# Shuijing725/CrowdNav_Prediction_AttnGraph

Hardware: NVIDIA H100
Metric: env_steps_per_s_ppo_rollout (higher is better)
Workload: dtype f32

## Files before the change

### crowdnav_prediction_attngraph_b200/_capi.py

```python
import ctypes as C
import os

_PKG = os.path.dirname(os.path.abspath(__file__))
LIB_PATH = os.path.join(_PKG, "libcrowdnav_b200.so")


class CnConfig(C.Structure):
    _fields_ = [(n, C.c_int32) for n in (
        "num_envs", "nenv_total", "rank_offset", "seed", "human_num", "predict_steps", "const_vel",
        "randomize_attributes", "random_goal_changing", "end_goal_changing", "sort_humans", "device",
        "phase", "val_size", "test_size", "human_num_range", "human_policy")] + \
        [("robot_policy", C.c_int16), ("robot_visible", C.c_int16)] + \
        [(n, C.c_double) for n in (
            "time_step", "time_limit", "pred_timestep", "circle_radius", "arena_size",
            "discomfort_dist", "discomfort_penalty_factor", "success_reward", "collision_penalty",
            "human_radius", "human_v_pref", "human_fov", "robot_radius", "robot_v_pref", "robot_fov",
            "sensor_range", "goal_change_chance", "orca_neighbor_dist", "orca_safety_space",
            "orca_time_horizon", "sf_A", "sf_B", "sf_KI")]


class CnObsPtrs(C.Structure):
    _fields_ = [("robot_node", C.c_void_p), ("temporal_edges", C.c_void_p), ("spatial_edges", C.c_void_p),
                ("detected_human_num", C.c_void_p), ("visible_masks", C.c_void_p)]

# ... 13 lines not shown


class CnActPtrs(C.Structure):
    _fields_ = [(n, C.c_void_p) for n in (
        "robot_node", "temporal_edges", "spatial_edges", "detected_human_num", "h_in", "masks", "noise",
        "value", "action", "log_prob", "h_out", "action_mean")]


class CnDsrnnConfig(C.Structure):
    _fields_ = [("num_envs", C.c_int32), ("human_num", C.c_int32), ("input_size", C.c_int32), ("device", C.c_int32)]


class CnDsrnnActPtrs(C.Structure):
    _fields_ = [(n, C.c_void_p) for n in (
        "robot_node", "temporal_edges", "spatial_edges", "h_in", "edge_h_in", "masks", "noise",
        "value", "action", "log_prob", "h_out", "edge_h_out", "action_mean")]


ABI_VERSION = 3

EXPORTS = [
    "cn_last_error", "cn_abi_version", "cn_env_create", "cn_env_destroy", "cn_env_reset", "cn_env_step",
    "cn_env_step_host", "cn_env_state_bytes", "cn_env_state_copy", "cn_env_launch_count", "cn_env_profile", "cn_env_stage_ms",
    "cn_policy_create", "cn_policy_destroy", "cn_policy_set_param", "cn_policy_finalize",
    "cn_policy_act", "cn_policy_launch_count", "cn_policy_last_rows", "cn_policy_profile", "cn_policy_stage_count",
    "cn_policy_stage_name", "cn_policy_handle_stage_name", "cn_policy_stage_ms", "cn_copy_segments", "cn_fetch_sync",
    "cn_gst_create", "cn_gst_destroy", "cn_gst_set_param", "cn_gst_finalize", "cn_gst_reset", "cn_gst_step",
    "cn_gst_launch_count",
    "cn_update_linear_saved_bytes", "cn_update_linear_ws_bytes", "cn_update_linear_fwd", "cn_update_linear_bwd",
    "cn_update_attn_fwd", "cn_update_attn_bwd", "cn_update_gru_fwd", "cn_update_gru_bwd",
    "cn_dsrnn_create", "cn_dsrnn_destroy", "cn_dsrnn_set_param", "cn_dsrnn_finalize", "cn_dsrnn_act",
    "cn_dsrnn_launch_count", "cn_dsrnn_profile", "cn_dsrnn_stage_count", "cn_dsrnn_stage_name", "cn_dsrnn_stage_ms",
    "cn_env_create_collect", "cn_env_reset_collect", "cn_env_step_collect", "cn_recorder_create", "cn_recorder_destroy",
    "cn_recorder_append", "cn_recorder_pending", "cn_recorder_flush", "cn_write_rows_txt", "cn_format_rows",
]

_lib = None


def config_from_dict(d):
    cfg = CnConfig()
    for name, _ in CnConfig._fields_:
        setattr(cfg, name, d[name])
    return cfg


# ... 40 lines not shown
    lib.cn_gst_create.restype = C.c_int
    lib.cn_gst_create.argtypes = [C.c_int, C.c_int, C.c_int, C.c_double, C.c_double, C.c_double, C.c_int, C.POINTER(C.c_void_p)]
    lib.cn_gst_destroy.argtypes = [C.c_void_p]
    lib.cn_gst_set_param.restype = C.c_int
    lib.cn_gst_set_param.argtypes = [C.c_void_p, C.c_char_p, C.c_void_p, C.c_size_t]
    lib.cn_gst_finalize.restype = C.c_int
    lib.cn_gst_finalize.argtypes = [C.c_void_p]
    lib.cn_gst_reset.restype = C.c_int
    lib.cn_gst_reset.argtypes = [C.c_void_p, C.c_void_p]
    lib.cn_gst_step.restype = C.c_int
    lib.cn_gst_step.argtypes = [C.c_void_p] * 7 + [C.c_void_p]
    lib.cn_gst_launch_count.restype = C.c_int64
    lib.cn_gst_launch_count.argtypes = [C.c_void_p]
    lib.cn_copy_segments.restype = C.c_int
    lib.cn_copy_segments.argtypes = [C.POINTER(CnCopySeg), C.c_int, C.c_int, C.c_void_p]
    lib.cn_fetch_sync.restype = C.c_int
    lib.cn_fetch_sync.argtypes = [C.c_void_p, C.c_void_p, C.c_size_t, C.c_int, C.c_void_p]
    lib.cn_env_launch_count.restype = C.c_int64
    lib.cn_env_launch_count.argtypes = [C.c_void_p]
    lib.cn_env_profile.restype = C.c_int
    lib.cn_env_profile.argtypes = [C.c_void_p, C.c_int]
    lib.cn_env_stage_ms.restype = C.c_int
    lib.cn_env_stage_ms.argtypes = [C.c_void_p, C.POINTER(C.c_float)]
    lib.cn_policy_create.argtypes = [C.POINTER(CnPolicyConfig), C.POINTER(C.c_void_p)]
    lib.cn_policy_destroy.argtypes = [C.c_void_p]
    lib.cn_policy_set_param.argtypes = [C.c_void_p, C.c_char_p, C.c_void_p, C.c_size_t]
    lib.cn_policy_finalize.argtypes = [C.c_void_p, C.c_void_p]
    lib.cn_policy_act.argtypes = [C.c_void_p, C.POINTER(CnActPtrs), C.c_void_p]
    lib.cn_policy_launch_count.restype = C.c_int64
    lib.cn_policy_launch_count.argtypes = [C.c_void_p]
    lib.cn_policy_last_rows.restype = C.c_int64
    lib.cn_policy_last_rows.argtypes = [C.c_void_p]
    lib.cn_policy_profile.argtypes = [C.c_void_p, C.c_int]
    lib.cn_policy_stage_count.restype = C.c_int
    lib.cn_policy_stage_name.restype = C.c_char_p
    lib.cn_policy_stage_name.argtypes = [C.c_int]
    lib.cn_policy_handle_stage_name.restype = C.c_char_p
    lib.cn_policy_handle_stage_name.argtypes = [C.c_void_p, C.c_int]
    lib.cn_policy_stage_ms.argtypes = [C.c_void_p, C.c_void_p, C.c_int]
    lib.cn_dsrnn_create.argtypes = [C.POINTER(CnDsrnnConfig), C.POINTER(C.c_void_p)]
    lib.cn_dsrnn_destroy.argtypes = [C.c_void_p]
    lib.cn_dsrnn_set_param.argtypes = [C.c_void_p, C.c_char_p, C.c_void_p, C.c_size_t]
    lib.cn_dsrnn_finalize.argtypes = [C.c_void_p, C.c_void_p]
    lib.cn_dsrnn_act.argtypes = [C.c_void_p, C.POINTER(CnDsrnnActPtrs), C.c_void_p]
    lib.cn_dsrnn_launch_count.restype = C.c_int64
    lib.cn_dsrnn_launch_count.argtypes = [C.c_void_p]
# ... 40 lines not shown
```

### crowdnav_prediction_attngraph_b200/csrc/cn_env_kernels.cu

```cuda
#include <cuda_runtime.h>
#include <stdio.h>
#include <stdlib.h>
#include <string.h>
#include <string>
#include <vector>
#include <map>

#include "../../include/crowdnav_b200.h"
#include "cn_env_core.cuh"
#include "cn_host_util.h"

namespace {

struct EnvSmemLayout {
  size_t per_env;
  size_t off_dbl;
  size_t off_flt;
  size_t off_u8;
};

__host__ __device__ inline size_t align16(size_t x) { return (x + 15) & ~(size_t)15; }

__host__ __device__ inline EnvSmemLayout env_layout(int H, bool lean, bool sf = false) {
  EnvSmemLayout L;
// ... 54 lines not shown

__device__ __forceinline__ void cn_sf_obs_lookahead(const CnParams& p, CnEnvSh* s, int h, bool live, float* row) {
  const bool seen = live && s->visr[h] != 0;
  double spx = 0.0, spy = 0.0, swx = 0.0, swy = 0.0, pen = 0.0;
  if (live) { spx = s->px[h]; spy = s->py[h]; swx = s->wx[h]; swy = s->wy[h]; }
  for (int t = 1; t <= p.lookahead_steps; ++t) {
    __syncthreads();
    CnD2 v = {0.0, 0.0};
    if (live) v = cn_sf_velocity(p, *s, h, false);
    __syncthreads();
    if (live) {
      const double x = s->px[h] + v.x * p.time_step, y = s->py[h] + v.y * p.time_step;
      s->px[h] = x; s->py[h] = y; s->wx[h] = v.x; s->wy[h] = v.y;
      if (seen && t % p.pred_interval == 0) cn_truth_row(p, *s, x, y, t / p.pred_interval, row, pen);
    }
  }
  __syncthreads();
  if (live) {
    s->px[h] = spx; s->py[h] = spy; s->wx[h] = swx; s->wy[h] = swy;
    if (seen) s->t1[h] = pen;
  }
}

template <int MAXH, int MAXW, bool ROBOT, bool VIS, bool COLLECT = false, bool SFLA = false, bool TRUTH = false>
__global__ void __launch_bounds__(288, 2) cn_env_step_kernel(CnParams p, CnState g, const float* __restrict__ action,
                                                          CnObs ob, CnStepOut out, int epb, int line_cap, int mode) {
  extern __shared__ __align__(16) unsigned char smem[];
  const int H = p.H;
  const int le = threadIdx.x / H;
  const int h = threadIdx.x - le * H;
  const int e = (le < epb) ? g.perm[blockIdx.x * epb + le] : p.N;
  const bool active = (le < epb) && (e < p.N);
  const EnvSmemLayout L = env_layout(H, true, p.social_force != 0);
  CnEnvSh* s = nullptr;
  if (le < epb) {
    s = reinterpret_cast<CnEnvSh*>(smem + (size_t)le * L.per_env);
    if (h == 0 && e < p.N) env_view(smem + (size_t)le * L.per_env, L, H, true, g, e, p.social_force != 0);
  }
  __syncthreads();
  const int warp = threadIdx.x >> 5, lane = threadIdx.x & 31;
  float4* lines_smem = reinterpret_cast<float4*>(smem + align16((size_t)epb * L.per_env));
  const int lstride = epb * H;
  CnWarpLines W;
  W.smem0 = lines_smem + warp * 32;
  W.stride = lstride;
  W.cap = line_cap;
  W.ovf_stride = g.ovf_stride;
  W.ovf0 = reinterpret_cast<float4*>(g.line_ovf) + ((size_t)blockIdx.x * blockDim.x + warp * 32) * g.ovf_stride;
  const int half = lane >> 4;
  const CnCoop hco = {lane & 15, 16, nullptr, nullptr, half ? 0xffff0000u : 0x0000ffffu, half << 4};
  CnLineStore proj;
  proj.base = lines_smem + (size_t)line_cap * lstride + (size_t)(2 * warp + half) * H;
  proj.stride = 1; proj.cap = H; proj.ovf = nullptr;
  unsigned char* lp3_q = reinterpret_cast<unsigned char*>(lines_smem + (size_t)line_cap * lstride +
                                                          (size_t)(blockDim.x >> 4) * H);
  if (threadIdx.x == 0) { reinterpret_cast<int*>(lp3_q)[0] = 0; reinterpret_cast<int*>(lp3_q)[1] = 0; }
  const CnCoop co = {lane, 32, nullptr, nullptr};

  if (mode == 1) {
    if (active && h == 0) { s->done = 1; s->info = 0; s->reward = 0.0; s->reset_flag = 0; s->nvis = 0; s->goal_flag = 0; s->lp3_cost = 0; s->hn = 0; }
  } else if (active) {
    cn_phase_load<MAXH, ROBOT>(p, g, *s, e, h, mode == 3 ? nullptr : action);
  }
  __syncthreads();
  const bool live = active && h < s->hn;
  int* lp3_count = reinterpret_cast<int*>(lp3_q);
  int* lp3_head = lp3_count + 1;
  unsigned short* lp3_tasks = reinterpret_cast<unsigned short*>(lp3_count + 2);
  auto orca_solve = [&](bool lv, bool use_fov, CnF2& result, int& nl, int& fail) {
    nl = 0; fail = -1;
    float vmax = 0.0f;
    CnF2 pref = f2(0.0f, 0.0f);
    result = f2(0.0f, 0.0f);
    if (lv) cn_orca_build<MAXH, VIS>(p, g, *s, e, h, W.of(lane), nl, vmax, pref, use_fov, mode == 3 ? (uint8_t)2 : (uint8_t)1);
    __syncwarp();
    cn_orca_lp2_warp(hco, W, nl, vmax, pref, result, fail);
    if (fail >= 0) {
      s->nvx[h] = result.x; s->nvy[h] = result.y;
      reinterpret_cast<int*>(&s->t0[h])[0] = nl | (fail << 8);
      reinterpret_cast<float*>(&s->t0[h])[1] = vmax;
      lp3_tasks[atomicAdd(lp3_count, 1)] = (unsigned short)threadIdx.x;
    }
    __syncthreads();
    const int ntask = *lp3_count;
    for (;;) {
      int t = 0;
      if (hco.lane == 0) t = atomicAdd(lp3_head, 1);
      t = __shfl_sync(hco.mask, t, hco.base);
      if (t >= ntask) break;
      const int owner = lp3_tasks[t];
      const int ole = owner / H, oh = owner - ole * H;
      CnEnvSh* os = reinterpret_cast<CnEnvSh*>(smem + (size_t)ole * L.per_env);
      const int packed = reinterpret_cast<const int*>(&os->t0[oh])[0];
      const float ovmax = reinterpret_cast<const float*>(&os->t0[oh])[1];
      CnF2 ores = f2(os->nvx[oh], os->nvy[oh]);
      CnLineStore ol;
      ol.base = lines_smem + owner; ol.stride = lstride; ol.cap = line_cap;
      ol.ovf = reinterpret_cast<float4*>(g.line_ovf) + ((size_t)blockIdx.x * blockDim.x + owner) * g.ovf_stride;
      cn_lp3_coop(hco, ol, packed & 0xff, packed >> 8, ovmax, ores, proj);
      if (hco.lane == 0) { os->nvx[oh] = ores.x; os->nvy[oh] = ores.y; }
    }
    __syncthreads();
    if (fail >= 0) result = f2(s->nvx[h], s->nvy[h]);
    if (threadIdx.x == 0) { *lp3_count = 0; *lp3_head = 0; }
  };
  if (mode != 1 && p.social_force) {
    if (live) cn_sf_action<VIS>(p, g, *s, e, h);
    if (SFLA && (!TRUTH || p.test_phase)) cn_sf_lookahead(p, g, s, e, h, live);
  } else if (mode == 2) {
    if (live) {
      const size_t i = cn_idx(p, e, h);
      const int nlf = g.pre_nlf[i];
      cn_orca_finish(p, g, *s, e, h, f2(g.pre_vx[i], g.pre_vy[i]), nlf & 0xff, (nlf >> 8) - 1);
      if (g.sim_exists[i] >= 2) g.sim_exists[i] = 1;
    }
  } else if (mode != 1) {
    CnF2 result; int nl, fail;
    orca_solve(live, true, result, nl, fail);
    if (live && fail >= 0) atomicAdd(&s->lp3_cost, 1);
    if (mode == 3) {
      if (live) {
        const size_t i = cn_idx(p, e, h);
        g.pre_vx[i] = result.x; g.pre_vy[i] = result.y; g.pre_nlf[i] = nl | ((fail + 1) << 8);
      }
      __syncthreads();
      if (active && h == 0) g.lp_cost[e] = s->lp3_cost;
      return;
    }
    if (p.test_phase && !COLLECT) {
      double spx = 0, spy = 0, lx = 0, ly = 0;
      float svx = 0, svy = 0, lvx = 0, lvy = 0;
      bool vis_prev = false;
      if (live) {
        spx = s->px[h]; spy = s->py[h]; svx = s->vx[h]; svy = s->vy[h];
        lx = spx; ly = spy; lvx = svx; lvy = svy;
        vis_prev = g.vis[cn_idx(p, e, h)] != 0;
      }
      CnLookahead la; la.min_rd = INFINITY; la.pen = 0.0;
      CnF2 lres = f2(0.0f, 0.0f); int lnl = 0, lfail = -1;
      for (int t = 1; t <= p.lookahead_steps; ++t) {
        __syncthreads();
        if (live) {
          s->px[h] = lx; s->py[h] = ly; s->fx[h] = (float)lx; s->fy[h] = (float)ly; s->vx[h] = lvx; s->vy[h] = lvy;
        }
        __syncthreads();
        orca_solve(live, false, lres, lnl, lfail);
        lx = lx + (double)lres.x * p.time_step; ly = ly + (double)lres.y * p.time_step;
        lvx = lres.x; lvy = lres.y;
        if (live && t % p.pred_interval == 0) cn_lookahead_accumulate(p, *s, vis_prev, lx, ly, t / p.pred_interval, la);
      }
      __syncthreads();
      if (live) {
        s->px[h] = spx; s->py[h] = spy; s->fx[h] = (float)spx; s->fy[h] = (float)spy; s->vx[h] = svx; s->vy[h] = svy;
      }
      __syncthreads();
      if (live) {
        cn_orca_finish(p, g, *s, e, h, result, nl, fail);
        cn_orca_diag(p, g, e, h, lres, lnl, lfail);
        s->t0[h] = la.min_rd; s->t1[h] = la.pen;
      }
    } else if (live) {
      cn_orca_finish(p, g, *s, e, h, result, nl, fail);
    }
  }
  __syncthreads();
  if (mode != 1 && active && h == 0) {
    if (COLLECT) cn_collect_reward(p, g, *s, e, out);
    else cn_phase_reward(p, g, *s, e, out);
  }
  if (COLLECT && mode == 1 && active && h == 0) g.rgoal_due[e] = 0;
  __syncthreads();
  if (active) {
    if (s->done) cn_install_env(p, g, *s, e, h);
    else if (live) cn_phase_integrate(p, *s, h);
  }
  __syncthreads();
  if (p.hrange > 0) {
    if (mode != 1 && active && h == 0 && cn_add_remove_due(p, g, *s, e)) cn_phase_add_remove(p, g, *s, e);
    __syncthreads();
  }
  float row[MAXW];
  if (COLLECT) {
    __shared__ uint32_t leaving[(288 + 31) / 32];
    const bool seen_before = active && h < s->hn && g.vis[cn_idx(p, e, h)] != 0;
    if (active) cn_phase_obs_a<MAXW>(p, g, *s, e, h, row);
    __syncthreads();
    const uint32_t b = __ballot_sync(0xffffffffu, seen_before && !s->reset_flag && !s->visr[h]);
    if (lane == 0) leaving[warp] = b;
    __syncthreads();
    if (active) cn_collect_ids(p, g, *s, e, h, leaving, le * H, ob);
    __syncthreads();
    if (active) cn_phase_store(p, g, *s, e, h);
    if (active && h == 0) {
      cn_collect_ids_done(p, g, *s, e, leaving, le * H);
      int evt = cn_event_flag(p, g, *s, e);
      if (evt == 0 && g.rgoal_due[e]) evt = 1;
      g.evt[e] = (uint8_t)evt;
      if (mode != 2) g.lp_cost[e] = s->lp3_cost;
    }
// ... 25 lines not shown
        lvx = lres.x; lvy = lres.y;
        if (seen && t % p.pred_interval == 0) cn_truth_row(p, *s, lx, ly, t / p.pred_interval, row, pen);
      }
      __syncthreads();
      if (olive) {
        s->px[h] = spx; s->py[h] = spy; s->fx[h] = (float)spx; s->fy[h] = (float)spy; s->vx[h] = svx; s->vy[h] = svy;
        s->t0[h] = key;
        if (seen) s->t1[h] = pen;
        if (p.lookahead_steps > 0) cn_orca_diag(p, g, e, h, lres, lnl, lfail);
      }
    }
    __syncthreads();
  }
  if (active) cn_phase_obs_b(p, g, *s, e, h, row, ob);
  __syncthreads();
  if (active) {
    cn_phase_obs_c(p, *s, e, h, ob);
    cn_phase_store(p, g, *s, e, h);
  }
  if (active && h == 0) {
    g.evt[e] = (uint8_t)cn_event_flag(p, g, *s, e);
    if (mode != 2) g.lp_cost[e] = s->lp3_cost;
  }
}

#define CN_EVENT_WARPS 4
template <bool COLLECT = false>
__global__ void __launch_bounds__(CN_EVENT_WARPS * 32) cn_env_event_kernel(CnParams p, CnState g, int force,
                                                                           size_t per_warp_bytes) {
  extern __shared__ __align__(16) unsigned char smem[];
  const int warp = threadIdx.x >> 5, lane = threadIdx.x & 31;
  const int e = blockIdx.x * CN_EVENT_WARPS + warp;
  if (e >= p.N) return;
  const int evt = force ? 2 : g.evt[e];
  if (evt == 0) return;
  const int H = p.H;
  const EnvSmemLayout L = env_layout(H, false, p.social_force != 0);
  unsigned char* base = smem + (size_t)warp * per_warp_bytes;
  CnEnvSh* s = reinterpret_cast<CnEnvSh*>(base);
  if (lane == 0) env_view(base, L, H, false, g, e, p.social_force != 0);
  __syncwarp();
  uint32_t* key = reinterpret_cast<uint32_t*>(base + L.per_env);
  const CnCoop co = {lane, 32, nullptr, reinterpret_cast<float*>(key + 624)};
  bool deferred;
  if (evt == 2) {
    deferred = cn_prepare_env(p, g, *s, e, key, co, p.defer_tries);
// ... 95 lines not shown
  } else {
    const unsigned char* s1 = reinterpret_cast<const unsigned char*>(sg.src);
    unsigned char* d1 = reinterpret_cast<unsigned char*>(sg.dst);
    for (size_t i = tid; i < sg.bytes; i += nth) d1[i] = s1[i];
  }
}

struct Field {
  void* ptr;
  size_t bytes;
};

}

struct cn_env {
  cn_config cfg;
  CnParams p;
  CnState g;
  int device;
  int epb;
  int threads;
  size_t smem_bytes;
  int line_cap;
  size_t reset_warp_bytes;
  int heavy_grid;
  size_t heavy_smem;
  int maxh;
  int64_t launches;
  std::map<std::string, Field> fields;
  std::vector<void*> allocs;
  cudaStream_t side;
  cudaEvent_t ev_step, ev_side;
  bool profile = false;
  cudaEvent_t pev[5] = {nullptr, nullptr, nullptr, nullptr, nullptr};
  bool side_pending;
  bool use_side;
  bool presolve;
  bool presolved;
  bool balance;
  bool prep_dirty;
  float* d_action;
  cn_obs_ptrs d_obs;
  cn_step_ptrs d_out;
};

namespace {
// ... 33 lines not shown
}

KernelFn pick_kernel_sfla(int maxh) {
  if (maxh <= 32) return cn_env_step_kernel<32, 16, true, true, false, true>;
  if (maxh <= 64) return cn_env_step_kernel<64, 16, true, true, false, true>;
  return cn_env_step_kernel<128, 16, true, true, false, true>;
}

template <bool SF>
KernelFn pick_kernel_truth(int maxh) {
  if (maxh <= 32) return cn_env_step_kernel<32, 16, false, true, false, SF, true>;
  if (maxh <= 64) return cn_env_step_kernel<64, 16, false, true, false, SF, true>;
  return cn_env_step_kernel<128, 16, false, true, false, SF, true>;
}

KernelFn pick_kernel(const CnParams& p, int maxh) {
  if (p.collect) return pick_kernel_collect(maxh);
  if (p.const_vel == 2) return p.social_force ? pick_kernel_truth<true>(maxh) : pick_kernel_truth<false>(maxh);
  if (p.social_force && p.test_phase) return pick_kernel_sfla(maxh);
  const bool robot = p.robot_policy != 0, vis = p.robot_visible != 0;
  return vis ? pick_kernel_vis<true>(maxh, robot) : pick_kernel_vis<false>(maxh, robot);
}

CnObs to_obs(const cn_obs_ptrs* o) {
  CnObs ob;
  ob.robot_node = o->robot_node; ob.temporal_edges = o->temporal_edges; ob.spatial_edges = o->spatial_edges;
  ob.detected_human_num = o->detected_human_num; ob.visible_masks = o->visible_masks;
  ob.pred_info = nullptr;
  return ob;
}

int event_kernel(cn_env* env, int force, cudaStream_t stream) {
  const int grid = (env->p.N + CN_EVENT_WARPS - 1) / CN_EVENT_WARPS;
  if (env->p.collect)
    cn_env_event_kernel<true><<<grid, CN_EVENT_WARPS * 32, CN_EVENT_WARPS * env->reset_warp_bytes, stream>>>(
        env->p, env->g, force, env->reset_warp_bytes);
  else
    cn_env_event_kernel<<<grid, CN_EVENT_WARPS * 32, CN_EVENT_WARPS * env->reset_warp_bytes, stream>>>(
        env->p, env->g, force, env->reset_warp_bytes);
  env->launches += 1;
  cudaError_t err = cudaGetLastError();
  if (err != cudaSuccess) return cn_set_error("cn_env_event_kernel launch: %s", cudaGetErrorString(err));
  if (env->p.collect)
    cn_env_event_heavy_kernel<true><<<env->heavy_grid, CN_HEAVY_THREADS, env->heavy_smem, stream>>>(env->p, env->g);
  else
    cn_env_event_heavy_kernel<<<env->heavy_grid, CN_HEAVY_THREADS, env->heavy_smem, stream>>>(env->p, env->g);
// ... 6 lines not shown
int join_side(cn_env* env, cudaStream_t stream) {
  if (!env->side_pending) return 0;
  cudaError_t err = cudaStreamWaitEvent(stream, env->ev_side, 0);
  if (err != cudaSuccess) return cn_set_error("cudaStreamWaitEvent(side): %s", cudaGetErrorString(err));
  env->side_pending = false;
  return 0;
}

int launch_step(cn_env* env, const float* d_action, const cn_obs_ptrs* o, const cn_step_ptrs* r, int mode,
                cudaStream_t stream, float* d_pred_info = nullptr) {
  CnStepOut out;
  memset(&out, 0, sizeof(out));
  if (r) {
    out.reward = r->reward; out.done = r->done; out.info = r->info; out.info_aux = r->info_aux;
    out.ep_ret = r->ep_ret; out.ep_len = r->ep_len; out.not_done = r->not_done;
  }
  int rc = join_side(env, stream);
  if (rc) return rc;
  if (mode == 1 || env->prep_dirty) {
    rc = event_kernel(env, 1, stream);
    if (rc) return rc;
    env->prep_dirty = false;
  }
  const int grid = (env->p.N + env->epb - 1) / env->epb;
  KernelFn fn = pick_kernel(env->p, env->maxh);
  CnObs ob = to_obs(o);
  ob.pred_info = d_pred_info;
  const int kmode = (mode == 0 && env->presolved) ? 2 : mode;
  env->presolved = false;
  if (env->profile) cudaEventRecord(env->pev[0], stream);
  fn<<<grid, env->threads, env->smem_bytes, stream>>>(env->p, env->g, d_action, ob, out, env->epb, env->line_cap, kmode);
  if (env->profile) cudaEventRecord(env->pev[1], stream);
  env->launches += 1;
  cudaError_t err = cudaGetLastError();
  if (err != cudaSuccess) return cn_set_error("cn_env_step_kernel launch: %s", cudaGetErrorString(err));
  if (!env->use_side) return event_kernel(env, 0, stream);
  err = cudaEventRecord(env->ev_step, stream);
  if (err == cudaSuccess) err = cudaStreamWaitEvent(env->side, env->ev_step, 0);
  if (err != cudaSuccess) return cn_set_error("fork to side stream: %s", cudaGetErrorString(err));
  if (env->profile) cudaEventRecord(env->pev[2], env->side);
  rc = event_kernel(env, 0, env->side);
  if (rc) return rc;
  if (env->balance && mode == 0) {
    cn_env_balance_kernel<<<1, 1024, 0, env->side>>>(env->p, env->g, grid, env->epb);
    env->launches += 1;
  }
  if (env->profile) cudaEventRecord(env->pev[3], env->side);
  if (env->presolve) {
    fn<<<grid, env->threads, env->smem_bytes, env->side>>>(env->p, env->g, nullptr, ob, out, env->epb, env->line_cap, 3);
    env->launches += 1;
    err = cudaGetLastError();
    if (err != cudaSuccess) return cn_set_error("cn_env_step_kernel (pre-solve) launch: %s", cudaGetErrorString(err));
    env->presolved = true;
  }
  if (env->profile) cudaEventRecord(env->pev[4], env->side);
  err = cudaEventRecord(env->ev_side, env->side);
  if (err != cudaSuccess) return cn_set_error("cudaEventRecord(side): %s", cudaGetErrorString(err));
  env->side_pending = true;
  return 0;
}

}

extern "C" {

int cn_abi_version(void) { return CN_ABI_VERSION; }

}

namespace {

int env_create(const cn_config* cfg, cn_env** out, bool collect) {
  if (!cfg || !out) return cn_set_error("cn_env_create: null argument");
  *out = nullptr;
  if (cfg->num_envs <= 0 || cfg->human_num <= 0 || cfg->human_num_range < 0 || cfg->human_num_range >= cfg->human_num ||
      cfg->human_num + cfg->human_num_range > 128)
    return cn_set_error("cn_env_create: need num_envs > 0, 0 <= human_num_range < human_num and human_num + range <= 128 "
                        "(got %d, %d, %d)", cfg->num_envs, cfg->human_num, cfg->human_num_range);
  if (cfg->const_vel < 0 || cfg->const_vel > 2)
    return cn_set_error("cn_env_create: const_vel %d unsupported (0 = CrowdSimVarNum-v0, 1 = CrowdSimPred-v0 'const_vel', "
                        "2 = CrowdSimPred-v0 'truth')", cfg->const_vel);
  if (cfg->const_vel && (cfg->predict_steps < 0 || 2 * (cfg->predict_steps + 1) > 16))
    return cn_set_error("cn_env_create: predict_steps %d unsupported (row width > 16)", cfg->predict_steps);
  {
    const double ts = cfg->time_step * 1024.0;
    if (!(cfg->time_step > 0) || ts != floor(ts))
      return cn_set_error("cn_env_create: time_step %.17g is not a multiple of 1/1024 (the engine keeps global_time as "
                          "step * time_step, exact only for such steps)", cfg->time_step);
  }
  int ndev = 0;
  cudaError_t err = cudaGetDeviceCount(&ndev);
  if (err != cudaSuccess || ndev == 0)
    return cn_set_error("cn_env_create: no CUDA device (%s); this engine has no CPU fallback",
                        err == cudaSuccess ? "device count 0" : cudaGetErrorString(err));
  if (cfg->device < 0 || cfg->device >= ndev) return cn_set_error("cn_env_create: bad device %d", cfg->device);
  err = cudaSetDevice(cfg->device);
  if (err != cudaSuccess) return cn_set_error("cudaSetDevice: %s", cudaGetErrorString(err));

  cn_env* env = new cn_env();
  env->cfg = *cfg;
  env->device = cfg->device;
  env->launches = 0;
  env->side = nullptr; env->ev_step = nullptr; env->ev_side = nullptr;
  env->side_pending = false; env->prep_dirty = true;
  {
    const char* ns = getenv("CN_NO_SIDE_STREAM");
    env->use_side = !(ns && ns[0] == '1');
    const char* ps = getenv("CN_PRESOLVE");
    const bool want = ps ? ps[0] != '0' : (cfg->human_num + cfg->human_num_range <= 32);
    env->presolve = env->use_side && want && cfg->human_policy == 0 && cfg->phase != 2 && cfg->const_vel != 2;
    env->presolved = false;
  }
  err = cudaStreamCreateWithFlags(&env->side, cudaStreamNonBlocking);
  if (err == cudaSuccess) err = cudaEventCreateWithFlags(&env->ev_step, cudaEventDisableTiming);
  if (err == cudaSuccess) err = cudaEventCreateWithFlags(&env->ev_side, cudaEventDisableTiming);
  if (err != cudaSuccess) { cn_env_destroy(env); return cn_set_error("side stream: %s", cudaGetErrorString(err)); }
  CnParams& p = env->p;
  memset(&p, 0, sizeof(p));
  p.hbase = cfg->human_num; p.hrange = cfg->human_num_range;
  p.N = cfg->num_envs; p.H = cfg->human_num + cfg->human_num_range; p.P = cfg->predict_steps;
  p.const_vel = cfg->const_vel;
  p.W = p.const_vel ? 2 * (p.P + 1) : 2;
  p.randomize = cfg->randomize_attributes; p.goal_changing = cfg->random_goal_changing;
  p.end_goal_changing = cfg->end_goal_changing; p.sort_humans = cfg->sort_humans;
  p.nenv_total = cfg->nenv_total; p.seed_base = (uint32_t)(cfg->seed + cfg->rank_offset);
  p.time_step = cfg->time_step; p.time_limit = cfg->time_limit;
  {
    const double q = floor(cfg->pred_timestep / cfg->time_step);
    p.pred_dt = cfg->time_step * (double)(int)q;
  }
  if (cfg->human_policy != 0 && cfg->human_policy != 1) {
    cn_env_destroy(env);
// ... 80 lines not shown
    if (err != cudaSuccess) rc = cn_set_error("init seed_off: %s", cudaGetErrorString(err));
  }
  memset(&env->d_obs, 0, sizeof(env->d_obs)); memset(&env->d_out, 0, sizeof(env->d_out));
  env->d_action = nullptr;
  if (!rc) rc = dev_alloc(env, nullptr, &env->d_action, N * 2);
  if (!rc) rc = dev_alloc(env, nullptr, &env->d_obs.robot_node, N * 7);
  if (!rc) rc = dev_alloc(env, nullptr, &env->d_obs.temporal_edges, N * 2);
  if (!rc) rc = dev_alloc(env, nullptr, &env->d_obs.spatial_edges, NH * p.W);
  if (!rc) rc = dev_alloc(env, nullptr, &env->d_obs.detected_human_num, N);
  if (!rc && !p.const_vel) rc = dev_alloc(env, nullptr, &env->d_obs.visible_masks, NH);
  if (!rc) rc = dev_alloc(env, nullptr, &env->d_out.reward, N);
  if (!rc) rc = dev_alloc(env, nullptr, &env->d_out.done, N);
  if (!rc) rc = dev_alloc(env, nullptr, &env->d_out.info, N);
  if (!rc) rc = dev_alloc(env, nullptr, &env->d_out.info_aux, N);
  if (!rc) rc = dev_alloc(env, nullptr, &env->d_out.ep_ret, N);
  if (!rc) rc = dev_alloc(env, nullptr, &env->d_out.ep_len, N);
  env->d_out.not_done = nullptr;
  if (rc) { cn_env_destroy(env); return rc; }

  env->maxh = p.H <= 32 ? 32 : (p.H <= 64 ? 64 : 128);
  const EnvSmemLayout L = env_layout(p.H, true, p.social_force != 0);
  int nsm = 0;
  cudaDeviceGetAttribute(&nsm, cudaDevAttrMultiProcessorCount, cfg->device);
  KernelFn fn = pick_kernel(p, env->maxh);
  size_t smem_cap = 227 * 1024;
  {
    cudaFuncAttributes fa;
    err = cudaFuncGetAttributes(&fa, fn);
    if (err != cudaSuccess) { cn_env_destroy(env); return cn_set_error("cudaFuncGetAttributes: %s", cudaGetErrorString(err)); }
    smem_cap -= fa.sharedSizeBytes;
  }
  err = cudaFuncSetAttribute(fn, cudaFuncAttributeMaxDynamicSharedMemorySize, (int)smem_cap);
  if (err != cudaSuccess) { cn_env_destroy(env); return cn_set_error("cudaFuncSetAttribute: %s", cudaGetErrorString(err)); }
  const int max_lines = p.H - 1 + p.robot_visible;
  const int cap_max = max_lines > 1 ? max_lines : 1;
  int best_epb = 0, best_cap = 0, best_threads = 0;
  size_t best_need = 0;
  bool best_single = false;
  for (int epb = 288 / p.H > 0 ? 288 / p.H : 1; epb >= 1; --epb) {
    const int threads = ((epb * p.H + 31) / 32) * 32;
    if (threads > 288) continue;
    const int grid_try = (p.N + epb - 1) / epb;
    for (int cap = cap_max; cap >= 1; --cap) {
      const size_t need = align16((size_t)epb * L.per_env) + (size_t)cap * epb * p.H * sizeof(float4) +
                          (size_t)(threads / 16) * p.H * sizeof(float4) +
                          align16(8 + 2 * (size_t)threads);
      if (need > smem_cap) continue;
      int per_sm = 0;
      err = cudaOccupancyMaxActiveBlocksPerMultiprocessor(&per_sm, fn, threads, need);
      if (err != cudaSuccess) { cn_env_destroy(env); return cn_set_error("occupancy query: %s", cudaGetErrorString(err)); }
      const bool single = (long long)per_sm * nsm >= grid_try;
      const bool better = !best_epb || (single && !best_single) ||
                          (single == best_single && (cap > best_cap || (cap == best_cap && epb > best_epb)));
      if (better && (single || !best_single)) {
        best_epb = epb; best_cap = cap; best_threads = threads; best_need = need; best_single = single;
      }
      if (single) break;
    }
  }
  if (!best_epb) { cn_env_destroy(env); return cn_set_error("cn_env_create: human_num %d does not fit shared memory", p.H); }
  env->epb = best_epb; env->threads = best_threads; env->line_cap = best_cap; env->smem_bytes = best_need;
  const int grid = (p.N + env->epb - 1) / env->epb;
  {
    float4* ovf = nullptr;
    env->g.ovf_stride = (max_lines - env->line_cap) > 0 ? (max_lines - env->line_cap) : 1;
    int rc2 = dev_alloc(env, nullptr, &ovf, (size_t)grid * env->threads * env->g.ovf_stride);
    if (rc2) { cn_env_destroy(env); return rc2; }
    env->g.line_ovf = ovf;
  }
  {
    int* perm = nullptr;
    int rc3 = dev_alloc(env, nullptr, &perm, (size_t)grid * env->epb);
    if (rc3) { cn_env_destroy(env); return rc3; }
    std::vector<int> id((size_t)grid * env->epb);
    for (size_t i = 0; i < id.size(); ++i) id[i] = (int)i;
    err = cudaMemcpy(perm, id.data(), id.size() * sizeof(int), cudaMemcpyHostToDevice);
    if (err != cudaSuccess) { cn_env_destroy(env); return cn_set_error("init perm: %s", cudaGetErrorString(err)); }
    env->g.perm = perm;
    const char* nb = getenv("CN_NO_BALANCE");
    env->balance = !(nb && nb[0] == '1') && env->use_side;
  }
  env->reset_warp_bytes = align16(env_layout(p.H, false, p.social_force != 0).per_env + 624 * sizeof(uint32_t) + 5 * CN_FTAB * sizeof(float));
  err = collect ? cudaFuncSetAttribute(cn_env_event_kernel<true>, cudaFuncAttributeMaxDynamicSharedMemorySize,
                                       (int)(CN_EVENT_WARPS * env->reset_warp_bytes))
                : cudaFuncSetAttribute(cn_env_event_kernel<false>, cudaFuncAttributeMaxDynamicSharedMemorySize,
                                       (int)(CN_EVENT_WARPS * env->reset_warp_bytes));
  if (err != cudaSuccess) { cn_env_destroy(env); return cn_set_error("cudaFuncSetAttribute(reset): %s", cudaGetErrorString(err)); }
  env->heavy_smem = align16(env_layout(p.H, false, p.social_force != 0).per_env + 624 * sizeof(uint32_t) + 64 + 5 * CN_FTAB * sizeof(float));
  {
    int sms = 132;
    cudaDeviceGetAttribute(&sms, cudaDevAttrMultiProcessorCount, cfg->device);
    env->heavy_grid = sms / 2 > 0 ? sms / 2 : 1;
    if (env->heavy_grid > p.N) env->heavy_grid = p.N;
  }
  err = collect ? cudaFuncSetAttribute(cn_env_event_heavy_kernel<true>, cudaFuncAttributeMaxDynamicSharedMemorySize,
                                       (int)env->heavy_smem)
                : cudaFuncSetAttribute(cn_env_event_heavy_kernel<false>, cudaFuncAttributeMaxDynamicSharedMemorySize,
                                       (int)env->heavy_smem);
  if (err != cudaSuccess) { cn_env_destroy(env); return cn_set_error("cudaFuncSetAttribute(heavy): %s", cudaGetErrorString(err)); }
  *out = env;
  return 0;
// ... 158 lines not shown
      if (cudaEventCreate(&env->pev[i]) != cudaSuccess) return cn_set_error("cn_env_profile: cudaEventCreate failed");
  }
  env->profile = enable != 0;
  return 0;
}

int cn_env_stage_ms(cn_env* env, float* out3) {
  if (!env || !out3) return cn_set_error("cn_env_stage_ms: null argument");
  if (!env->pev[0]) return cn_set_error("cn_env_stage_ms: call cn_env_profile(env, 1) before the step");
  CnDeviceGuard guard(env->device);
  cudaError_t err = cudaDeviceSynchronize();
  out3[0] = out3[1] = out3[2] = 0.0f;
  if (err == cudaSuccess) err = cudaEventElapsedTime(&out3[0], env->pev[0], env->pev[1]);
  if (err == cudaSuccess && env->use_side) {
    err = cudaEventElapsedTime(&out3[1], env->pev[2], env->pev[3]);
    if (err == cudaSuccess) err = cudaEventElapsedTime(&out3[2], env->pev[3], env->pev[4]);
  }
  if (err != cudaSuccess) return cn_set_error("cn_env_stage_ms: %s", cudaGetErrorString(err));
  return 0;
}

int64_t cn_env_launch_count(cn_env* env) { return env ? env->launches : 0; }

}
```

### include/crowdnav_b200.h

```cpp
#ifndef CROWDNAV_B200_H
#define CROWDNAV_B200_H

#include <stddef.h>
#include <stdint.h>

#ifdef __cplusplus
extern "C" {
#endif

#define CN_ABI_VERSION 3

#define CN_INFO_NOTHING_C 0
#define CN_INFO_TIMEOUT_C 1
#define CN_INFO_COLLISION_C 2
#define CN_INFO_REACHGOAL_C 3
#define CN_INFO_DANGER_C 4

typedef struct cn_config {
  int32_t num_envs;
  int32_t nenv_total;
  int32_t rank_offset;
  int32_t seed;
  int32_t human_num;
  int32_t predict_steps;
// ... 59 lines not shown

typedef struct cn_env cn_env;

const char *cn_last_error(void);
int cn_abi_version(void);

int cn_env_create(const cn_config *cfg, cn_env **out);
int cn_env_destroy(cn_env *env);

int cn_env_reset(cn_env *env, const cn_obs_ptrs *d_obs, void *stream);

int cn_env_step(cn_env *env, const float *d_action, const cn_obs_ptrs *d_obs,
                const cn_step_ptrs *d_out, void *stream);

int cn_env_step_host(cn_env *env, const float *h_action, const cn_obs_ptrs *h_obs,
                     const cn_step_ptrs *h_out);

size_t cn_env_state_bytes(cn_env *env, const char *name);
int cn_env_state_copy(cn_env *env, const char *name, void *h_buf, size_t bytes, int dir);

int64_t cn_env_launch_count(cn_env *env);
int cn_env_profile(cn_env *env, int enable);
int cn_env_stage_ms(cn_env *env, float *out3);

int cn_env_create_collect(const cn_config *cfg, cn_env **out);
int cn_env_reset_collect(cn_env *env, float *d_pred_info, void *stream);
int cn_env_step_collect(cn_env *env, const float *d_action, float *d_pred_info, const cn_step_ptrs *d_out, void *stream);

typedef struct cn_recorder cn_recorder;
int cn_recorder_create(int num_envs, int human_num, int chunk_frames, int device, cn_recorder **out);
int cn_recorder_destroy(cn_recorder *r);
int cn_recorder_append(cn_recorder *r, const float *d_pred_info, void *stream);
int cn_recorder_pending(cn_recorder *r);
int cn_recorder_flush(cn_recorder *r, float *h_rows, int64_t *h_env_rows, int64_t *n_rows, void *stream);
int cn_write_rows_txt(const char *dir, const float *h_rows, const int64_t *h_env_rows, int num_envs, int env_base,
                      int append);
int64_t cn_format_rows(const float *h_rows, int64_t n, char *out, int64_t cap);


typedef struct cn_policy cn_policy;

typedef struct cn_policy_config {
  int32_t num_envs;
  int32_t human_num;
  int32_t input_size;
  int32_t device;
// ... 91 lines not shown
```

Before: 6.802 million.

## Specialize presolve and finish env kernels with separate launch shapes

Splits the single env step kernel into compile-time specialized variants for pre-solve and the finishing pass. Each variant gets its own occupancy-driven launch shape: the finish pass needs no line buffers, so it can pack more envs per SM, and it uses identity slots instead of the balance permutation. The default presolve threshold is raised from 32 to 64 humans, and optional tracing hooks are added behind a compile flag. This adds more template instantiations and separate slot and overflow buffers, and the balance kernel now follows the pre-solve shape.

New measurement: 6.829 million (median of 6 runs). No clear change (+0.4%).

```diff
diff --git a/crowdnav_prediction_attngraph_b200/_capi.py b/crowdnav_prediction_attngraph_b200/_capi.py
--- a/crowdnav_prediction_attngraph_b200/_capi.py
+++ b/crowdnav_prediction_attngraph_b200/_capi.py
@@ -59,6 +59,7 @@
 EXPORTS = [
     "cn_last_error", "cn_abi_version", "cn_env_create", "cn_env_destroy", "cn_env_reset", "cn_env_step",
     "cn_env_step_host", "cn_env_state_bytes", "cn_env_state_copy", "cn_env_launch_count", "cn_env_profile", "cn_env_stage_ms",
+    "cn_env_launch_shape",
     "cn_policy_create", "cn_policy_destroy", "cn_policy_set_param", "cn_policy_finalize",
     "cn_policy_act", "cn_policy_launch_count", "cn_policy_last_rows", "cn_policy_profile", "cn_policy_stage_count",
     "cn_policy_stage_name", "cn_policy_handle_stage_name", "cn_policy_stage_ms", "cn_copy_segments", "cn_fetch_sync",
@@ -145,6 +146,8 @@
     lib.cn_env_profile.argtypes = [C.c_void_p, C.c_int]
     lib.cn_env_stage_ms.restype = C.c_int
     lib.cn_env_stage_ms.argtypes = [C.c_void_p, C.POINTER(C.c_float)]
+    lib.cn_env_launch_shape.restype = C.c_int
+    lib.cn_env_launch_shape.argtypes = [C.c_void_p, C.c_int, C.POINTER(C.c_int)]
     lib.cn_policy_create.argtypes = [C.POINTER(CnPolicyConfig), C.POINTER(C.c_void_p)]
     lib.cn_policy_destroy.argtypes = [C.c_void_p]
     lib.cn_policy_set_param.argtypes = [C.c_void_p, C.c_char_p, C.c_void_p, C.c_size_t]
diff --git a/crowdnav_prediction_attngraph_b200/csrc/cn_env_kernels.cu b/crowdnav_prediction_attngraph_b200/csrc/cn_env_kernels.cu
--- a/crowdnav_prediction_attngraph_b200/csrc/cn_env_kernels.cu
+++ b/crowdnav_prediction_attngraph_b200/csrc/cn_env_kernels.cu
@@ -100,14 +100,47 @@
   }
 }
 
-template <int MAXH, int MAXW, bool ROBOT, bool VIS, bool COLLECT = false, bool SFLA = false, bool TRUTH = false>
-__global__ void __launch_bounds__(288, 2) cn_env_step_kernel(CnParams p, CnState g, const float* __restrict__ action,
-                                                          CnObs ob, CnStepOut out, int epb, int line_cap, int mode) {
+#define CN_KIND_STEP 0
+#define CN_KIND_PRESOLVE 1
+#define CN_KIND_FINISH 2
+#ifdef CN_ENV_TRACE
+#define CN_TRACE_REC 10
+#define CN_TRACE_FIN_CTA 65536
+__device__ unsigned long long* cn_env_trace_buf = nullptr;
+__device__ __forceinline__ unsigned long long cn_gtimer() {
+  unsigned long long t;
+  asm volatile("mov.u64 %0, %%globaltimer;" : "=l"(t));
+  return t;
+}
+__device__ __forceinline__ unsigned cn_smid() {
+  unsigned r;
+  asm volatile("mov.u32 %0, %%smid;" : "=r"(r));
+  return r;
+}
+#define CN_TRACE_REC_PTR(k) \
+  (cn_env_trace_buf + (size_t)(blockIdx.x + (KIND == CN_KIND_FINISH ? CN_TRACE_FIN_CTA : 0)) * CN_TRACE_REC + (k))
+#define CN_TRACE_T(k) do { if (cn_env_trace_buf && threadIdx.x == 0) *CN_TRACE_REC_PTR(k) = cn_gtimer(); } while (0)
+#define CN_TRACE_WMAX(k) do { if (cn_env_trace_buf && (threadIdx.x & 31) == 0) atomicMax(CN_TRACE_REC_PTR(k), cn_gtimer()); } while (0)
+#define CN_TRACE_ADD(k, v) do { if (cn_env_trace_buf && (v)) atomicAdd(CN_TRACE_REC_PTR(k), (unsigned long long)(v)); } while (0)
+#define CN_TRACE_SET(k, v) do { if (cn_env_trace_buf && threadIdx.x == 0) *CN_TRACE_REC_PTR(k) = (unsigned long long)(v); } while (0)
+#else
+#define CN_TRACE_T(k) do { } while (0)
+#define CN_TRACE_WMAX(k) do { } while (0)
+#define CN_TRACE_ADD(k, v) do { } while (0)
+#define CN_TRACE_SET(k, v) do { } while (0)
+#endif
+template <int MAXH, int MAXW, bool ROBOT, bool VIS, bool COLLECT = false, bool SFLA = false, bool TRUTH = false,
+          int KIND = CN_KIND_STEP>
+__global__ void __launch_bounds__(288, KIND == CN_KIND_STEP ? 2 : 3)
+cn_env_step_kernel(CnParams p, CnState g, const float* __restrict__ action, CnObs ob, CnStepOut out, int epb, int line_cap,
+                   int mode_arg) {
   extern __shared__ __align__(16) unsigned char smem[];
+  const int mode = KIND == CN_KIND_PRESOLVE ? 3 : (KIND == CN_KIND_FINISH ? 2 : mode_arg);
+  CN_TRACE_T(0);
   const int H = p.H;
   const int le = threadIdx.x / H;
   const int h = threadIdx.x - le * H;
-  const int e = (le < epb) ? g.perm[blockIdx.x * epb + le] : p.N;
+  const int e = (le < epb) ? (KIND == CN_KIND_FINISH ? blockIdx.x * epb + le : g.perm[blockIdx.x * epb + le]) : p.N;
   const bool active = (le < epb) && (e < p.N);
   const EnvSmemLayout L = env_layout(H, true, p.social_force != 0);
   CnEnvSh* s = nullptr;
@@ -132,8 +165,7 @@
   proj.stride = 1; proj.cap = H; proj.ovf = nullptr;
   unsigned char* lp3_q = reinterpret_cast<unsigned char*>(lines_smem + (size_t)line_cap * lstride +
                                                           (size_t)(blockDim.x >> 4) * H);
-  if (threadIdx.x == 0) { reinterpret_cast<int*>(lp3_q)[0] = 0; reinterpret_cast<int*>(lp3_q)[1] = 0; }
-  const CnCoop co = {lane, 32, nullptr, nullptr};
+  if (KIND != CN_KIND_FINISH && threadIdx.x == 0) { reinterpret_cast<int*>(lp3_q)[0] = 0; reinterpret_cast<int*>(lp3_q)[1] = 0; }
 
   if (mode == 1) {
     if (active && h == 0) { s->done = 1; s->info = 0; s->reward = 0.0; s->reset_flag = 0; s->nvis = 0; s->goal_flag = 0; s->lp3_cost = 0; s->hn = 0; }
@@ -141,6 +173,7 @@
     cn_phase_load<MAXH, ROBOT>(p, g, *s, e, h, mode == 3 ? nullptr : action);
   }
   __syncthreads();
+  CN_TRACE_T(1);
   const bool live = active && h < s->hn;
   int* lp3_count = reinterpret_cast<int*>(lp3_q);
   int* lp3_head = lp3_count + 1;
@@ -152,7 +185,10 @@
     result = f2(0.0f, 0.0f);
     if (lv) cn_orca_build<MAXH, VIS>(p, g, *s, e, h, W.of(lane), nl, vmax, pref, use_fov, mode == 3 ? (uint8_t)2 : (uint8_t)1);
     __syncwarp();
+    CN_TRACE_WMAX(2);
+    CN_TRACE_ADD(7, nl > line_cap ? nl - line_cap : 0);
     cn_orca_lp2_warp(hco, W, nl, vmax, pref, result, fail);
+    CN_TRACE_WMAX(3);
     if (fail >= 0) {
       s->nvx[h] = result.x; s->nvy[h] = result.y;
       reinterpret_cast<int*>(&s->t0[h])[0] = nl | (fail << 8);
@@ -161,6 +197,7 @@
     }
     __syncthreads();
     const int ntask = *lp3_count;
+    CN_TRACE_SET(8, ntask);
     for (;;) {
       int t = 0;
       if (hco.lane == 0) t = atomicAdd(lp3_head, 1);
@@ -179,10 +216,11 @@
       if (hco.lane == 0) { os->nvx[oh] = ores.x; os->nvy[oh] = ores.y; }
     }
     __syncthreads();
+    CN_TRACE_T(4);
     if (fail >= 0) result = f2(s->nvx[h], s->nvy[h]);
     if (threadIdx.x == 0) { *lp3_count = 0; *lp3_head = 0; }
   };
-  if (mode != 1 && p.social_force) {
+  if (KIND == CN_KIND_STEP && mode != 1 && p.social_force) {
     if (live) cn_sf_action<VIS>(p, g, *s, e, h);
     if (SFLA && (!TRUTH || p.test_phase)) cn_sf_lookahead(p, g, s, e, h, live);
   } else if (mode == 2) {
@@ -203,6 +241,8 @@
       }
       __syncthreads();
       if (active && h == 0) g.lp_cost[e] = s->lp3_cost;
+      CN_TRACE_T(5);
+      CN_TRACE_SET(9, cn_smid());
       return;
     }
     if (p.test_phase && !COLLECT) {
@@ -248,11 +288,13 @@
   }
   if (COLLECT && mode == 1 && active && h == 0) g.rgoal_due[e] = 0;
   __syncthreads();
+  if (KIND == CN_KIND_FINISH) CN_TRACE_T(2);
   if (active) {
     if (s->done) cn_install_env(p, g, *s, e, h);
     else if (live) cn_phase_integrate(p, *s, h);
   }
   __syncthreads();
+  if (KIND == CN_KIND_FINISH) CN_TRACE_T(3);
   if (p.hrange > 0) {
     if (mode != 1 && active && h == 0 && cn_add_remove_due(p, g, *s, e)) cn_phase_add_remove(p, g, *s, e);
     __syncthreads();
@@ -324,6 +366,11 @@
     g.evt[e] = (uint8_t)cn_event_flag(p, g, *s, e);
     if (mode != 2) g.lp_cost[e] = s->lp3_cost;
   }
+  if (KIND == CN_KIND_FINISH) {
+    __syncthreads();
+    CN_TRACE_T(4);
+    CN_TRACE_SET(9, cn_smid());
+  }
 }
 
 #define CN_EVENT_WARPS 4
@@ -465,6 +512,11 @@
   int threads;
   size_t smem_bytes;
   int line_cap;
+  int pre_epb, pre_threads, pre_line_cap;
+  size_t pre_smem_bytes;
+  int fin_epb, fin_threads;
+  size_t fin_smem_bytes;
+  int* step_slots;
   size_t reset_warp_bytes;
   int heavy_grid;
   size_t heavy_smem;
@@ -544,6 +596,33 @@
   return vis ? pick_kernel_vis<true>(maxh, robot) : pick_kernel_vis<false>(maxh, robot);
 }
 
+KernelFn pick_kernel_presolve(const CnParams& p, int maxh) {
+  if (p.collect || p.robot_visible) {
+    if (maxh <= 32) return cn_env_step_kernel<32, 16, false, true, false, false, false, CN_KIND_PRESOLVE>;
+    if (maxh <= 64) return cn_env_step_kernel<64, 16, false, true, false, false, false, CN_KIND_PRESOLVE>;
+    return cn_env_step_kernel<128, 16, false, true, false, false, false, CN_KIND_PRESOLVE>;
+  }
+  if (maxh <= 32) return cn_env_step_kernel<32, 16, false, false, false, false, false, CN_KIND_PRESOLVE>;
+  if (maxh <= 64) return cn_env_step_kernel<64, 16, false, false, false, false, false, CN_KIND_PRESOLVE>;
+  return cn_env_step_kernel<128, 16, false, false, false, false, false, CN_KIND_PRESOLVE>;
+}
+
+KernelFn pick_kernel_finish(const CnParams& p, int maxh) {
+  if (p.collect) {
+    if (maxh <= 32) return cn_env_step_kernel<32, 16, true, false, true, false, false, CN_KIND_FINISH>;
+    if (maxh <= 64) return cn_env_step_kernel<64, 16, true, false, true, false, false, CN_KIND_FINISH>;
+    return cn_env_step_kernel<128, 16, true, false, true, false, false, CN_KIND_FINISH>;
+  }
+  if (p.robot_policy != 0) {
+    if (maxh <= 32) return cn_env_step_kernel<32, 16, true, false, false, false, false, CN_KIND_FINISH>;
+    if (maxh <= 64) return cn_env_step_kernel<64, 16, true, false, false, false, false, CN_KIND_FINISH>;
+    return cn_env_step_kernel<128, 16, true, false, false, false, false, CN_KIND_FINISH>;
+  }
+  if (maxh <= 32) return cn_env_step_kernel<32, 16, false, false, false, false, false, CN_KIND_FINISH>;
+  if (maxh <= 64) return cn_env_step_kernel<64, 16, false, false, false, false, false, CN_KIND_FINISH>;
+  return cn_env_step_kernel<128, 16, false, false, false, false, false, CN_KIND_FINISH>;
+}
+
 CnObs to_obs(const cn_obs_ptrs* o) {
   CnObs ob;
   ob.robot_node = o->robot_node; ob.temporal_edges = o->temporal_edges; ob.spatial_edges = o->spatial_edges;
@@ -596,14 +675,21 @@
     if (rc) return rc;
     env->prep_dirty = false;
   }
-  const int grid = (env->p.N + env->epb - 1) / env->epb;
-  KernelFn fn = pick_kernel(env->p, env->maxh);
   CnObs ob = to_obs(o);
   ob.pred_info = d_pred_info;
-  const int kmode = (mode == 0 && env->presolved) ? 2 : mode;
+  CnState gi = env->g;
+  if (env->presolve) gi.perm = env->step_slots;
+  if (env->profile) cudaEventRecord(env->pev[0], stream);
+  if (mode == 0 && env->presolved) {
+    const int grid = (env->p.N + env->fin_epb - 1) / env->fin_epb;
+    pick_kernel_finish(env->p, env->maxh)<<<grid, env->fin_threads, env->fin_smem_bytes, stream>>>(
+        env->p, gi, d_action, ob, out, env->fin_epb, 0, 2);
+  } else {
+    const int grid = (env->p.N + env->epb - 1) / env->epb;
+    pick_kernel(env->p, env->maxh)<<<grid, env->threads, env->smem_bytes, stream>>>(env->p, gi, d_action, ob, out,
+                                                                                    env->epb, env->line_cap, mode);
+  }
   env->presolved = false;
-  if (env->profile) cudaEventRecord(env->pev[0], stream);
-  fn<<<grid, env->threads, env->smem_bytes, stream>>>(env->p, env->g, d_action, ob, out, env->epb, env->line_cap, kmode);
   if (env->profile) cudaEventRecord(env->pev[1], stream);
   env->launches += 1;
   cudaError_t err = cudaGetLastError();
@@ -616,12 +702,15 @@
   rc = event_kernel(env, 0, env->side);
   if (rc) return rc;
   if (env->balance && mode == 0) {
-    cn_env_balance_kernel<<<1, 1024, 0, env->side>>>(env->p, env->g, grid, env->epb);
+    const int bepb = env->presolve ? env->pre_epb : env->epb;
+    cn_env_balance_kernel<<<1, 1024, 0, env->side>>>(env->p, env->g, (env->p.N + bepb - 1) / bepb, bepb);
     env->launches += 1;
   }
   if (env->profile) cudaEventRecord(env->pev[3], env->side);
   if (env->presolve) {
-    fn<<<grid, env->threads, env->smem_bytes, env->side>>>(env->p, env->g, nullptr, ob, out, env->epb, env->line_cap, 3);
+    const int pgrid = (env->p.N + env->pre_epb - 1) / env->pre_epb;
+    pick_kernel_presolve(env->p, env->maxh)<<<pgrid, env->pre_threads, env->pre_smem_bytes, env->side>>>(
+        env->p, env->g, nullptr, ob, out, env->pre_epb, env->pre_line_cap, 3);
     env->launches += 1;
     err = cudaGetLastError();
     if (err != cudaSuccess) return cn_set_error("cn_env_step_kernel (pre-solve) launch: %s", cudaGetErrorString(err));
@@ -643,6 +732,56 @@
 }
 
 namespace {
+
+struct Shape {
+  int epb, threads, cap;
+  size_t smem;
+};
+
+int prepare_kernel(KernelFn fn, size_t total) {
+  cudaFuncAttributes fa;
+  cudaError_t err = cudaFuncGetAttributes(&fa, fn);
+  if (err != cudaSuccess) return cn_set_error("cudaFuncGetAttributes: %s", cudaGetErrorString(err));
+  err = cudaFuncSetAttribute(fn, cudaFuncAttributeMaxDynamicSharedMemorySize, (int)(total - fa.sharedSizeBytes));
+  if (err != cudaSuccess) return cn_set_error("cudaFuncSetAttribute: %s", cudaGetErrorString(err));
+  return 0;
+}
+
+int search_solve_shape(KernelFn fn, int N, int H, const EnvSmemLayout& L, int nsm, int cap_max, int want_epb, int want_cap,
+                       Shape& out) {
+  cudaFuncAttributes fa;
+  cudaError_t err = cudaFuncGetAttributes(&fa, fn);
+  if (err != cudaSuccess) return cn_set_error("cudaFuncGetAttributes: %s", cudaGetErrorString(err));
+  const size_t smem_cap = (size_t)fa.maxDynamicSharedSizeBytes;
+  int best_epb = 0, best_cap = 0, best_threads = 0;
+  size_t best_need = 0;
+  bool best_single = false;
+  for (int epb = 288 / H > 0 ? 288 / H : 1; epb >= 1; --epb) {
+    const int threads = ((epb * H + 31) / 32) * 32;
+    if (threads > 288 || (want_epb > 0 && epb != want_epb)) continue;
+    const int grid_try = (N + epb - 1) / epb;
+    for (int cap = want_cap > 0 ? want_cap : cap_max; cap >= 1; --cap) {
+      const size_t need = align16((size_t)epb * L.per_env) + (size_t)cap * epb * H * sizeof(float4) +
+                          (size_t)(threads / 16) * H * sizeof(float4) +
+                          align16(8 + 2 * (size_t)threads);
+      if (need > smem_cap) continue;
+      int per_sm = 0;
+      err = cudaOccupancyMaxActiveBlocksPerMultiprocessor(&per_sm, fn, threads, need);
+      if (err != cudaSuccess) return cn_set_error("occupancy query: %s", cudaGetErrorString(err));
+      if (per_sm < 1) continue;
+      const bool single = (long long)per_sm * nsm >= grid_try;
+      const bool better = !best_epb || (single && !best_single) ||
+                          (single == best_single && (cap > best_cap || (cap == best_cap && epb > best_epb)));
+      if (better && (single || !best_single)) {
+        best_epb = epb; best_cap = cap; best_threads = threads; best_need = need; best_single = single;
+      }
+      if (single || want_cap > 0) break;
+    }
+  }
+  if (!best_epb) return cn_set_error("cn_env_create: human_num %d does not fit shared memory", H);
+  out.epb = best_epb; out.threads = best_threads; out.cap = best_cap; out.smem = best_need;
+  return 0;
+}
 
 int env_create(const cn_config* cfg, cn_env** out, bool collect) {
   if (!cfg || !out) return cn_set_error("cn_env_create: null argument");
@@ -681,7 +820,7 @@
     const char* ns = getenv("CN_NO_SIDE_STREAM");
     env->use_side = !(ns && ns[0] == '1');
     const char* ps = getenv("CN_PRESOLVE");
-    const bool want = ps ? ps[0] != '0' : (cfg->human_num + cfg->human_num_range <= 32);
+    const bool want = ps ? ps[0] != '0' : (cfg->human_num + cfg->human_num_range <= 64);
     env->presolve = env->use_side && want && cfg->human_policy == 0 && cfg->phase != 2 && cfg->const_vel != 2;
     env->presolved = false;
   }
@@ -808,61 +947,77 @@
   const EnvSmemLayout L = env_layout(p.H, true, p.social_force != 0);
   int nsm = 0;
   cudaDeviceGetAttribute(&nsm, cudaDevAttrMultiProcessorCount, cfg->device);
-  KernelFn fn = pick_kernel(p, env->maxh);
-  size_t smem_cap = 227 * 1024;
+  const int max_lines = p.H - 1 + p.robot_visible;
+  int cap_max = max_lines > 1 ? max_lines : 1;
   {
-    cudaFuncAttributes fa;
-    err = cudaFuncGetAttributes(&fa, fn);
-    if (err != cudaSuccess) { cn_env_destroy(env); return cn_set_error("cudaFuncGetAttributes: %s", cudaGetErrorString(err)); }
-    smem_cap -= fa.sharedSizeBytes;
-  }
-  err = cudaFuncSetAttribute(fn, cudaFuncAttributeMaxDynamicSharedMemorySize, (int)smem_cap);
-  if (err != cudaSuccess) { cn_env_destroy(env); return cn_set_error("cudaFuncSetAttribute: %s", cudaGetErrorString(err)); }
-  const int max_lines = p.H - 1 + p.robot_visible;
-  const int cap_max = max_lines > 1 ? max_lines : 1;
-  int best_epb = 0, best_cap = 0, best_threads = 0;
-  size_t best_need = 0;
-  bool best_single = false;
-  for (int epb = 288 / p.H > 0 ? 288 / p.H : 1; epb >= 1; --epb) {
-    const int threads = ((epb * p.H + 31) / 32) * 32;
-    if (threads > 288) continue;
-    const int grid_try = (p.N + epb - 1) / epb;
-    for (int cap = cap_max; cap >= 1; --cap) {
-      const size_t need = align16((size_t)epb * L.per_env) + (size_t)cap * epb * p.H * sizeof(float4) +
-                          (size_t)(threads / 16) * p.H * sizeof(float4) +
-                          align16(8 + 2 * (size_t)threads);
-      if (need > smem_cap) continue;
+    const char* lc = getenv("CN_LINE_CAP");
+    if (lc && atoi(lc) >= 1 && atoi(lc) < cap_max) cap_max = atoi(lc);
+  }
+  Shape shp;
+  rc = prepare_kernel(pick_kernel(p, env->maxh), 227 * 1024);
+  if (!rc) rc = search_solve_shape(pick_kernel(p, env->maxh), p.N, p.H, L, nsm, cap_max, 0, 0, shp);
+  if (rc) { cn_env_destroy(env); return rc; }
+  env->epb = shp.epb; env->threads = shp.threads; env->line_cap = shp.cap; env->smem_bytes = shp.smem;
+  int min_cap = env->line_cap;
+  size_t ovf_threads = (size_t)((p.N + env->epb - 1) / env->epb) * env->threads;
+  size_t perm_slots = (size_t)((p.N + env->epb - 1) / env->epb) * env->epb;
+  env->pre_epb = env->pre_threads = env->pre_line_cap = 0; env->pre_smem_bytes = 0;
+  env->fin_epb = env->fin_threads = 0; env->fin_smem_bytes = 0;
+  if (env->presolve) {
+    int want_epb = 0, want_cap = 0;
+    const char* sh = getenv("CN_PRESOLVE_SHAPE");
+    if (sh) sscanf(sh, "%d,%d", &want_epb, &want_cap);
+    KernelFn pfn = pick_kernel_presolve(p, env->maxh);
+    rc = prepare_kernel(pfn, 227 * 1024);
+    if (!rc) rc = search_solve_shape(pfn, p.N, p.H, L, nsm, cap_max, want_epb, want_cap < cap_max ? want_cap : cap_max, shp);
+    if (rc) { cn_env_destroy(env); return rc; }
+    env->pre_epb = shp.epb; env->pre_threads = shp.threads; env->pre_line_cap = shp.cap; env->pre_smem_bytes = shp.smem;
+    if (shp.cap < min_cap) min_cap = shp.cap;
+    const size_t pgrid = (size_t)((p.N + shp.epb - 1) / shp.epb);
+    if (pgrid * shp.threads > ovf_threads) ovf_threads = pgrid * shp.threads;
+    perm_slots = pgrid * shp.epb;
+    KernelFn ffn = pick_kernel_finish(p, env->maxh);
+    rc = prepare_kernel(ffn, 227 * 1024);
+    if (rc) { cn_env_destroy(env); return rc; }
+    long long best = -1;
+    for (int epb = 288 / p.H > 0 ? 288 / p.H : 1; epb >= 1; --epb) {
+      const int threads = ((epb * p.H + 31) / 32) * 32;
+      if (threads > 288) continue;
+      const size_t need = align16((size_t)epb * L.per_env);
       int per_sm = 0;
-      err = cudaOccupancyMaxActiveBlocksPerMultiprocessor(&per_sm, fn, threads, need);
+      err = cudaOccupancyMaxActiveBlocksPerMultiprocessor(&per_sm, ffn, threads, need);
       if (err != cudaSuccess) { cn_env_destroy(env); return cn_set_error("occupancy query: %s", cudaGetErrorString(err)); }
-      const bool single = (long long)per_sm * nsm >= grid_try;
-      const bool better = !best_epb || (single && !best_single) ||
-                          (single == best_single && (cap > best_cap || (cap == best_cap && epb > best_epb)));
-      if (better && (single || !best_single)) {
-        best_epb = epb; best_cap = cap; best_threads = threads; best_need = need; best_single = single;
-      }
-      if (single) break;
-    }
-  }
-  if (!best_epb) { cn_env_destroy(env); return cn_set_error("cn_env_create: human_num %d does not fit shared memory", p.H); }
-  env->epb = best_epb; env->threads = best_threads; env->line_cap = best_cap; env->smem_bytes = best_need;
-  const int grid = (p.N + env->epb - 1) / env->epb;
+      const long long grid_f = (p.N + epb - 1) / epb;
+      const long long resident = (long long)per_sm * nsm < grid_f ? (long long)per_sm * nsm * epb : (long long)p.N;
+      if (resident > best) { best = resident; env->fin_epb = epb; env->fin_threads = threads; env->fin_smem_bytes = need; }
+    }
+  }
   {
     float4* ovf = nullptr;
-    env->g.ovf_stride = (max_lines - env->line_cap) > 0 ? (max_lines - env->line_cap) : 1;
-    int rc2 = dev_alloc(env, nullptr, &ovf, (size_t)grid * env->threads * env->g.ovf_stride);
+    env->g.ovf_stride = (max_lines - min_cap) > 0 ? (max_lines - min_cap) : 1;
+    int rc2 = dev_alloc(env, nullptr, &ovf, ovf_threads * env->g.ovf_stride);
     if (rc2) { cn_env_destroy(env); return rc2; }
     env->g.line_ovf = ovf;
   }
   {
     int* perm = nullptr;
-    int rc3 = dev_alloc(env, nullptr, &perm, (size_t)grid * env->epb);
+    int rc3 = dev_alloc(env, nullptr, &perm, perm_slots);
     if (rc3) { cn_env_destroy(env); return rc3; }
-    std::vector<int> id((size_t)grid * env->epb);
+    std::vector<int> id(perm_slots);
     for (size_t i = 0; i < id.size(); ++i) id[i] = (int)i;
     err = cudaMemcpy(perm, id.data(), id.size() * sizeof(int), cudaMemcpyHostToDevice);
     if (err != cudaSuccess) { cn_env_destroy(env); return cn_set_error("init perm: %s", cudaGetErrorString(err)); }
     env->g.perm = perm;
+    env->step_slots = perm;
+    if (env->presolve) {
+      const size_t slots = (size_t)((p.N + env->epb - 1) / env->epb) * env->epb;
+      std::vector<int> sid(slots);
+      for (size_t i = 0; i < slots; ++i) sid[i] = (int)i;
+      rc3 = dev_alloc(env, nullptr, &env->step_slots, slots);
+      if (rc3) { cn_env_destroy(env); return rc3; }
+      err = cudaMemcpy(env->step_slots, sid.data(), slots * sizeof(int), cudaMemcpyHostToDevice);
+      if (err != cudaSuccess) { cn_env_destroy(env); return cn_set_error("init step slots: %s", cudaGetErrorString(err)); }
+    }
     const char* nb = getenv("CN_NO_BALANCE");
     env->balance = !(nb && nb[0] == '1') && env->use_side;
   }
@@ -1067,4 +1222,24 @@
 
 int64_t cn_env_launch_count(cn_env* env) { return env ? env->launches : 0; }
 
-}
+int cn_env_launch_shape(cn_env* env, int kind, int* out4) {
+  if (!env || !out4) return cn_set_error("cn_env_launch_shape: null argument");
+  if (kind < 0 || kind > 2) return cn_set_error("cn_env_launch_shape: kind %d (0 = step, 1 = pre-solve, 2 = finishing pass)", kind);
+  if (kind && !env->presolve) return cn_set_error("cn_env_launch_shape: this handle runs no pre-solve");
+  const int epb[3] = {env->epb, env->pre_epb, env->fin_epb};
+  const int threads[3] = {env->threads, env->pre_threads, env->fin_threads};
+  const int cap[3] = {env->line_cap, env->pre_line_cap, 0};
+  const size_t smem[3] = {env->smem_bytes, env->pre_smem_bytes, env->fin_smem_bytes};
+  out4[0] = epb[kind]; out4[1] = threads[kind]; out4[2] = cap[kind]; out4[3] = (int)smem[kind];
+  return 0;
+}
+
+#ifdef CN_ENV_TRACE
+int cn_env_trace(unsigned long long* dbuf) {
+  cudaError_t err = cudaMemcpyToSymbol(cn_env_trace_buf, &dbuf, sizeof(dbuf));
+  if (err != cudaSuccess) return cn_set_error("cn_env_trace: %s", cudaGetErrorString(err));
+  return 0;
+}
+#endif
+
+}
diff --git a/include/crowdnav_b200.h b/include/crowdnav_b200.h
--- a/include/crowdnav_b200.h
+++ b/include/crowdnav_b200.h
@@ -105,6 +105,7 @@
 int64_t cn_env_launch_count(cn_env *env);
 int cn_env_profile(cn_env *env, int enable);
 int cn_env_stage_ms(cn_env *env, float *out3);
+int cn_env_launch_shape(cn_env *env, int kind, int *out4);
 
 int cn_env_create_collect(const cn_config *cfg, cn_env **out);
 int cn_env_reset_collect(cn_env *env, float *d_pred_info, void *stream);
```
